# MCV-Univalle/HM-OpenCL

Hardware: AMD Instinct MI355X
Metric: GSAD/s (higher is better)
Workload: dtype u8

## Files before the change

### hm-opencl_amd/csrc/hmme.hip

```cpp
#include "../../include/hmme.h"
#include "../../include/hmme_test.h"

#include <hip/hip_runtime.h>

#include <climits>
#include <cmath>
#include <cstdarg>
#include <cstdio>
#include <cstdlib>
#include <cstring>
#include <functional>
#include <string>
#include <type_traits>
#include <vector>

#include "me_kernels.hpp"

using hmme::MeJob;
using hmme::MeJob16;
using hmme::RefSet;

namespace {
constexpr int kMarginX = 128;
constexpr int kMarginY = 80;
// ... 1225 lines not shown
    const int h = hmme::me_strip_rows16(w, w, rmax, n_min + 4);
    pl.n_strips = (w + h - 1) / h;
    const int lanes = (((w + 1) >> 1) + 2) / 3;
    auto strip_cost = [&](int k) {
      const int hk = (w + k - 1) / k;
      return 2.0 * ((((hk * lanes + 63) >> 6) + 3) >> 2) + 1.0;
    };
    if (tail && knobs.tail_parts != 1) {
      const int k_max = std::min(w / 4, 64);
      int k = knobs.tail_parts > 1 ? std::min(knobs.tail_parts, k_max) : plan_tail(tail, slots, pl.n_strips, k_max, strip_cost);
      if (k < pl.n_strips) k = pl.n_strips;
      if (k > pl.n_strips) { pl.tail_first = jobs - tail; pl.tail_parts = k; }
    }
    pl.n_wg16 = pl.tail_first * pl.n_strips + (jobs - pl.tail_first) * pl.tail_parts;
    pl.table_bytes = sizeof(MeJob16) * (size_t)pl.n_wg16;
  } else if (search_range > 64) {
    pl.mode = SearchMode::kTiles8;
    pl.table_bytes = sizeof(MeJob16) * (size_t)jobs * 4;
  } else {
    const int wgs = tail && knobs.tail_parts != 1 ? plan_tail8(tail, slots, w, knobs.tail_parts) : 0;
    if (wgs > 0) { pl.tail_first = jobs - tail; pl.tail_wgs = wgs; }
    const int head = pl.tail_first, n_tail = jobs - head;
    if (!n_tail) {
      pl.table_bytes = sizeof(MeJob) * (size_t)head;
    } else if (tail_one_launch(head, n_tail, knobs.tail_launches)) {
      pl.mode = SearchMode::kSegments8;
      pl.table_bytes = hmme::me_seg_table_bytes(head + wgs, jobs);
    } else {
      pl.mode = SearchMode::kHeadThenSegments8;
      pl.tail_jobs_off = (sizeof(MeJob) * (size_t)head + 255) & ~(size_t)255;
      pl.table_bytes = pl.tail_jobs_off + hmme::me_seg_table_bytes(wgs, n_tail);
    }
  }
  pl.first_strip = pl.mode != SearchMode::kWhole8;
  const size_t per_ref = n_refs > 0 ? (pl.table_bytes + n_refs - 1) / n_refs : pl.table_bytes;
  pl.table_grow = per_ref * hmme::kMaxRefs + 4096;
  return pl;
}
static FramePlan plan_launch(const hmme_ctx* ctx, const hmme_frame_params* fp, int count, int n_refs, bool force16 = false) {
  return plan_search(count * n_refs, n_refs, ctx->wg_slots, fp->search_range, fp->bit_depth > 8 || force16, knobs());
}

int hmme_test_tail_plan(int width, int height, int search_range, int n_pairs, int slots, int* out) {
  if (!out || width < 8 || height < 8 || width > 16384 || height > 16384 || search_range < 1 || search_range > 64 || n_pairs < 1 || slots < 1) return HMME_ERR_ARG;
  const FramePlan pl = plan_search(hmme_num_ctus(width, height) * n_pairs, n_pairs, slots, search_range, false, Knobs{});
  out[0] = pl.jobs; out[1] = pl.tail_first; out[2] = pl.tail_wgs; out[3] = pl.mode == SearchMode::kSegments8 ? 1 : 0;
  return HMME_OK;
}

int hmme_test_pk_gate(uint32_t lambda_q16) { return hmme::me_pk_gate(lambda_q16) ? 1 : 0; }
int hmme_test_pk_body(uint32_t lambda_q16, int fen) { return hmme::me_pk_body(lambda_q16, fen ? 1 : 0); }
int hmme_test_pk_task_marker_free(int wx, int wy, int k, int it0, int n_it) { return hmme::me_task_marker_free(wx, wy, k, it0, n_it) ? 1 : 0; }
int hmme_test_pk_task_full(int wx, int wy, int k, int it0, int n_it) { return hmme::me_task_full(wx, wy, k, it0, n_it) ? 1 : 0; }

static int prep_jobs(hmme_ctx* ctx, const hmme_plane* cur, const hmme_frame_params* fp, const void* d_pred_q, int first, int count,
                     int n_refs, hipStream_t s, const FramePlan& pl, const void* d_center_q = nullptr) {
  const int jobs = pl.jobs, head = pl.tail_first, n_tail = jobs - head, w = cur->width, h = cur->height, sr = fp->search_range;
  bool moved;
  int rc = ensure(ctx, ctx->buf[kJobs], pl.table_bytes, pl.table_grow, &moved);
  if (moved) ctx->jobs_tag.valid = false;
  if (rc) return rc;
  if (pl.first_strip) {
    rc = ensure(ctx, ctx->buf[kFirstStrip], sizeof(int) * (size_t)jobs, sizeof(int) * (size_t)(jobs / (n_refs > 0 ? n_refs : 1) + 1) * hmme::kMaxRefs, &moved);
    if (moved) ctx->jobs_tag.valid = false;
    if (rc) return rc;
  }
  void* const d_jobs = ctx->buf[kJobs].p;
  int* const d_first_strip = ctx->buf[kFirstStrip].as<int>();
  hmme_ctx::TableTag tag;
  tag.valid = !d_pred_q && !d_center_q;
  tag.w = w; tag.h = h; tag.sr = sr; tag.first = first; tag.count = count; tag.pairs = n_refs;
  tag.bit_depth = fp->bit_depth | (pl.mode == SearchMode::kStrips16 && fp->bit_depth == 8 ? 0x100 : 0);
  tag.buf = d_jobs; tag.buf2 = pl.first_strip ? d_first_strip : nullptr; tag.stream = (void*)s;
  if (tag.same(ctx->jobs_tag)) return HMME_OK;
  ctx->jobs_tag.valid = false;
  const dim3 block(256);
  const auto grid = [](int n) { return dim3((n + 255) / 256); };
  const int16_t* pred = (const int16_t*)d_pred_q;
  switch (pl.mode) {
    case SearchMode::kTiles8:
      hipLaunchKernelGGL(hmme::me_prep_jobs_tile_kernel, grid(jobs), block, 0, s, (MeJob16*)d_jobs, d_first_strip, pred, first, count, n_refs, w, h, sr);
      break;
    case SearchMode::kStrips16:
      hipLaunchKernelGGL(hmme::me_prep_jobs16_kernel, grid(jobs), block, 0, s, (MeJob16*)d_jobs, d_first_strip, pred, first, count, n_refs, w, h, sr,
                         pl.n_strips, pl.strip_rows, pl.tail_first, pl.tail_parts, (const int16_t*)d_center_q);
      break;
    case SearchMode::kWhole8:
    case SearchMode::kSegments8:
    case SearchMode::kHeadThenSegments8: {
      const int idx0 = pl.mode == SearchMode::kSegments8 ? head : 0;
      if (head && idx0)
        hipLaunchKernelGGL(hmme::me_prep_whole_segments_kernel, grid(head), block, 0, s, d_jobs, d_first_strip, pred, first, count, n_refs, w, h, sr,
                           head + pl.tail_wgs, head);
      else if (head)
        hipLaunchKernelGGL(hmme::me_prep_jobs_kernel, grid(head), block, 0, s, (MeJob*)d_jobs, pred, first, count, n_refs, w, h, sr, 0, head, 1,
                           (uint32_t*)nullptr, (const int16_t*)nullptr);
      if (n_tail)
        hipLaunchKernelGGL(hmme::me_prep_segments_kernel, dim3(1), dim3(hmme::kSegPrepThreads), 0, s, (void*)((uint8_t*)d_jobs + pl.tail_jobs_off), d_first_strip,
                           pred, first, count, n_refs, w, h, sr, idx0 + pl.tail_wgs, head, n_tail, idx0);
      break;
    }
  }
  HIP_TRY(ctx, hipGetLastError());
  ctx->jobs_tag = tag;
  return HMME_OK;
}
// ... 2671 lines not shown
```

### hm-opencl_amd/csrc/me_kernels.hpp

```cpp
#pragma once

#include <hip/hip_runtime.h>
#include <stdint.h>

namespace hmme {

constexpr int kParts = 593;
constexpr int kPDW = 49;
constexpr int kWinRowsMax = 192;
constexpr int kIdxBits = 10;
constexpr uint32_t kInvCost = 3146751u;
constexpr int kGroups = 10;
constexpr int kIterPerTask = 4;
constexpr int kIterPerTaskSplit = 1;
static_assert(kIterPerTask == 4 && kIterPerTaskSplit <= 4, "2 iteration bits in the key; the guided schedule deals 4 / 2 / 1");
constexpr int kThreads = 256;

struct MeJob {
  int16_t ctu_x, ctu_y;
  int16_t lt_x, lt_y;
  int16_t rb_x, rb_y;
  int16_t pred_x, pred_y;
};
static_assert(sizeof(MeJob) == 16, "MeJob layout");
// ... 35 lines not shown
  asm volatile("v_add3_u32 %0, %1, %2, %3" : "=v"(v##_3) : "v"(a##_3), "v"(b##_3), "v"(nc3))
#define ME_SUB(v, a, b)                                                                                         \
  uint32_t v##_0, v##_1, v##_2, v##_3;                                                                          \
  asm volatile("v_sad_u32 %0, %1, %2, %3" : "=v"(v##_0) : "v"(a##_0), "v"(b##_0), "v"(c0));                                \
  asm volatile("v_sad_u32 %0, %1, %2, %3" : "=v"(v##_1) : "v"(a##_1), "v"(b##_1), "v"(c1));                                \
  asm volatile("v_sad_u32 %0, %1, %2, %3" : "=v"(v##_2) : "v"(a##_2), "v"(b##_2), "v"(c2));                                \
  asm volatile("v_sad_u32 %0, %1, %2, %3" : "=v"(v##_3) : "v"(a##_3), "v"(b##_3), "v"(c3))
__device__ __forceinline__ uint32_t me_min4(uint32_t a, uint32_t b, uint32_t c, uint32_t d) {
  uint32_t r;
  asm volatile("v_min3_u32 %0, %1, %2, %3\n\tv_min_u32 %0, %0, %4" : "=&v"(r) : "v"(a), "v"(b), "v"(c), "v"(d));
  return r;
}
#define ME_MIN4(k) me_min4(k##_0, k##_1, k##_2, k##_3)
#define ME_SUBMIN4(r, a, b)                                                                                     \
  uint32_t r;                                                                                                   \
  {                                                                                                             \
    uint32_t r##_t, r##_u;                                                                                      \
    asm volatile("v_sad_u32 %0, %3, %7, %11\n\tv_sad_u32 %1, %4, %8, %12\n\tv_sad_u32 %2, %5, %9, %13\n\t"            \
                 "v_min3_u32 %0, %0, %1, %2\n\tv_sad_u32 %1, %6, %10, %14\n\tv_min_u32 %0, %0, %1"                    \
                 : "=&v"(r), "=&v"(r##_t), "=&v"(r##_u)                                                        \
                 : "v"(a##_0), "v"(a##_1), "v"(a##_2), "v"(a##_3), "v"(b##_0), "v"(b##_1), "v"(b##_2), "v"(b##_3), "v"(c0), "v"(c1),     \
                   "v"(c2), "v"(c3));                                                                           \
  }

constexpr uint32_t kPkSlotMax = 64 * 255;
constexpr uint32_t kPkMarker = 0xFFFFu - kPkSlotMax;
constexpr uint32_t kPkMaxBits = 2 * 37;
__host__ __device__ inline bool me_pk_gate(uint32_t lambda_q16) {
  const uint64_t prod = (uint64_t)lambda_q16 * kPkMaxBits;
  return prod <= 0xFFFFFFFFull && (prod >> 16) + kPkSlotMax < kPkMarker;
}
constexpr uint32_t kPk2SlotMax = 16 * 12 * 255;
__host__ __device__ inline bool me_pk2_gate(uint32_t lambda_q16) {
  const uint64_t prod = (uint64_t)lambda_q16 * kPkMaxBits;
  return prod <= 0xFFFFFFFFull && (prod >> 16) + kPk2SlotMax <= 0xFFFFu;
}
__host__ __device__ inline int me_pk_body(uint32_t lambda_q16, int fen) {
  return (fen && me_pk2_gate(lambda_q16)) ? 2 : me_pk_gate(lambda_q16) ? 1 : 0;
}
__host__ __device__ inline bool me_task_marker_free(int wx, int wy, int k, int it0, int n_it) {
  if (!(wx & 3)) return true;
  const int quads = (wx + 3) >> 2;
  if ((quads & -quads) == (1 << k)) return false;
  const bool fold = (quads & 32) && (quads & 31) && (wy & 1);
  return !(fold && k == 5 && 2 * (it0 + n_it) > wy);
}
__host__ __device__ inline bool me_task_full(int wx, int wy, int k, int it0, int n_it) {
  if (k < 2) return false;
  const int quads = (wx + 3) >> 2;
  if ((wx & 3) && (quads & -quads) == (1 << k)) return false;
  const bool fold = (quads & 32) && (quads & 31) && (wy & 1);
  return (it0 + n_it) * (64 >> k) <= ((k == 5 || !fold) ? wy : wy - 1);
}
#define ME_PKMIN(r, p) ME_PKMIN_Q(r, (p) + pkm)
#define ME_PKMINE(r, p) ME_PKMIN_Q(r, ((p) << 1) + pkm)
#define ME_PKMIN_Q(r, q)                                                                                        \
  uint32_t r;                                                                                                   \
  {                                                                                                             \
    const uint64_t r##_q = (q);                                                                                 \
    asm volatile("v_pk_min_u16 %0, %1, %2\n\tv_pk_min_u16 %0, %0, %0 op_sel:[0,1] op_sel_hi:[1,0]\n\t"                \
                 "v_mad_u32_u16 %0, %0, %3, %4"                                                                 \
                 : "=&v"(r) : "v"((uint32_t)r##_q), "v"((uint32_t)(r##_q >> 32)), "s"(mult_a), "v"(ctag));      \
  }

#define ME_PKMIN16_LO(r, q)                                                                                     \
  uint32_t r;                                                                                                   \
  {                                                                                                             \
    const uint64_t r##_q = (q);                                                                                 \
    asm volatile("v_pk_min_u16 %0, %1, %2\n\t"                                                                  \
                 "v_min_u16_sdwa %0, %0, %0 dst_sel:WORD_0 dst_unused:UNUSED_PAD src0_sel:WORD_0 src1_sel:WORD_1" \
                 : "=&v"(r) : "v"((uint32_t)r##_q), "v"((uint32_t)(r##_q >> 32)));                              \
  }
#define ME_PKMIN16_HI(r, q)                                                                                     \
  {                                                                                                             \
    const uint64_t r##_q = (q);                                                                                 \
    uint32_t r##_t;                                                                                             \
    asm volatile("v_pk_min_u16 %1, %2, %3\n\t"                                                                  \
                 "v_min_u16_sdwa %0, %1, %1 dst_sel:WORD_1 dst_unused:UNUSED_PRESERVE src0_sel:WORD_0 src1_sel:WORD_1" \
                 : "+v"(r), "=&v"(r##_t) : "v"((uint32_t)r##_q), "v"((uint32_t)(r##_q >> 32)));                 \
  }
#define ME_KEY16_LO(k, r) uint32_t k; asm volatile("v_mad_u32_u16 %0, %1, %2, %3" : "=v"(k) : "v"(r), "s"(mult_a), "v"(ctag))
#define ME_KEY16_HI(k, r) uint32_t k; asm volatile("v_mad_u32_u16 %0, %1, %2, %3 op_sel:[1,0,0,0]" : "=v"(k) : "v"(r), "s"(mult_a), "v"(ctag))
#define ME_PMERGE(NAME, PAD, SWAP)                                                                           \
  __device__ __forceinline__ uint32_t NAME(uint32_t a, uint32_t b) {                                         \
    asm volatile(PAD SWAP " %0, %1\n\tv_pk_min_u16 %0, %0, %1" : "+v"(a), "+v"(b));                          \
    return a;                                                                                                \
  }
ME_PMERGE(me_pmerge2, "s_nop 1\n\t", "v_permlane32_swap_b32")
ME_PMERGE(me_pmerge3, "s_nop 1\n\t", "v_permlane16_swap_b32")
ME_PMERGE(me_pmerge2_nn, "", "v_permlane32_swap_b32")
ME_PMERGE(me_pmerge3_nn, "", "v_permlane16_swap_b32")

#define ME_MERGE_DPP_MASKED(NAME, PAD, CTRL, MASK0)                                                          \
  __device__ __forceinline__ uint32_t NAME(uint32_t a, uint32_t b) {                                         \
    uint32_t r;                                                                                              \
    asm volatile(PAD "v_min_u32_dpp %0, %2, %2 " CTRL " row_mask:0xf bank_mask:0xf\n\t"                     \
        "v_min_u32_dpp %0, %1, %1 " CTRL " row_mask:0xf bank_mask:" MASK0                                    \
        : "=&v"(r) : "v"(a), "v"(b));                                                                        \
    return r;                                                                                                \
  }
ME_MERGE_DPP_MASKED(me_merge0, "s_nop 1\n\t", "row_ror:8", "0x3")
ME_MERGE_DPP_MASKED(me_merge1, "s_nop 1\n\t", "row_half_mirror", "0x5")
ME_MERGE_DPP_MASKED(me_merge0_nn, "", "row_ror:8", "0x3")
ME_MERGE_DPP_MASKED(me_merge1_nn, "", "row_half_mirror", "0x5")
__device__ __forceinline__ uint32_t me_merge2(uint32_t a, uint32_t b) {
  u32x2_t r = __builtin_amdgcn_permlane32_swap(a, b, false, false);
  return min(r.x, r.y);
}
__device__ __forceinline__ uint32_t me_merge3(uint32_t a, uint32_t b) {
  u32x2_t r = __builtin_amdgcn_permlane16_swap(a, b, false, false);
  return min(r.x, r.y);
}
template <int DPP_CTRL>
__device__ __forceinline__ uint32_t me_merge_dpp(uint32_t a, uint32_t b, bool role) {
  const uint32_t keep = role ? b : a;
  const uint32_t give = role ? a : b;
  return min(keep, (uint32_t)__builtin_amdgcn_update_dpp(0, (int)give, DPP_CTRL, 0xf, 0xf, false));
}
#define me_merge4(a, b, role) me_merge_dpp<0x4E>(a, b, role)
#define me_merge5(a, b, role) me_merge_dpp<0xB1>(a, b, role)

__device__ __forceinline__ uint32_t me_component_bits(int v) {
  const uint32_t t = (v <= 0) ? ((uint32_t)(-v) << 1) + 1u : ((uint32_t)v << 1);
  return 2u * (31u - (uint32_t)__builtin_clz(t)) + 1u;
}
__device__ __forceinline__ uint32_t me_mv_cost(uint32_t lambda_q16, int x, int y, int pred_x, int pred_y) {
  return (lambda_q16 * (me_component_bits((x << 2) - pred_x) + me_component_bits((y << 2) - pred_y))) >> 16;
}

__device__ __forceinline__ bool me_pk_slot(int s, bool wide, int& x, int& y, int& w, int& h) {
  if (s < 128) { x = (s & 7) * 8; y = (s >> 4) * 8 + ((s >> 3) & 1) * 4; w = 8; h = 4; return true; }
  if (s < 256) { x = ((s >> 1) & 7) * 8 + (s & 1) * 4; y = ((s - 128) >> 4) * 8; w = 4; h = 8; return true; }
  if (s >= 384 && s < 448) { x = (s & 7) * 8; y = ((s - 384) >> 3) * 8; w = 8; h = 8; return true; }
  if (!wide) return false;
  if (s < 384) {
    const int kk = (s - 256) >> 4;
    x = (s & 3) * 16; y = ((s >> 2) & 3) * 16; w = 16; h = 16;
    if (kk < 4) { h = kk < 2 ? 4 : 12; if (kk & 1) y += 16 - h; }
    else { w = kk < 6 ? 4 : 12; if (kk & 1) x += 16 - w; }
    return true;
  }
  if (s < 480) { x = (s & 3) * 16; y = ((s - 448) >> 3) * 16 + ((s >> 2) & 1) * 8; w = 16; h = 8; return true; }
  if (s < 512) { x = ((s >> 1) & 3) * 16 + (s & 1) * 8; y = ((s - 480) >> 3) * 16; w = 8; h = 16; return true; }
  return false;
}
template <int RW, int NR, int STEP>
__device__ __forceinline__ void me_pk_sads(const uint32_t* wrow, int pdw, const uint8_t* __restrict__ crow, uint32_t sad[4]) {
  constexpr int ND = RW / 4;
  static_assert(RW * NR * 255 <= 0xFFFF, "the four sums are packed u16");
  typedef uint64_t __attribute__((aligned(4))) u64a4_t;
  uint32_t c[NR][ND];
  uint64_t d[NR][ND];
#pragma unroll
  for (int r = 0; r < NR; ++r) {
#pragma unroll
    for (int k = 0; k < ND; ++k) c[r][k] = *(const uint32_t*)(crow + r * STEP * 64 + 4 * k);
#pragma unroll
    for (int k = 0; k < ND; ++k) d[r][k] = *(const u64a4_t*)(wrow + r * STEP * pdw + k);
  }
  uint64_t acc = 0;
#pragma unroll
  for (int r = 0; r < NR; ++r)
#pragma unroll
    for (int k = 0; k < ND; ++k) acc = ME_QSAD(d[r][k], c[r][k], acc);
#pragma unroll
  for (int j = 0; j < 4; ++j) sad[j] = (uint32_t)(acc >> (16 * j)) & 0xFFFFu;
}
template <bool WIDE>
__device__ __forceinline__ unsigned long long me_pk_recover(unsigned long long v, int s, const uint32_t* win, int pdw, const uint8_t* __restrict__ cur_blk,
                                                            const MeJob& job, int wx, uint32_t lambda_q16) {
  int rx, ry, rw, rh;
  if (v == ~0ull || !me_pk_slot(s, WIDE, rx, ry, rw, rh)) return v;
  const int x_first = (int)(v & 0xfffc), y = (int)((v >> 16) & 0xffff);
  const uint32_t cost = (uint32_t)(v >> 32);
  const uint8_t* crow = cur_blk + ry * 64 + rx;
  const uint32_t by = me_component_bits(((job.lt_y + y) << 2) - job.pred_y);
  const int x_end = (WIDE && !(x_first & 12)) ? min(x_first + 16, wx) : x_first + 4;
// ... 169 lines not shown
    if (!first_job) __syncthreads();
  }
  if (fair_prio) __builtin_amdgcn_s_setprio(3);
  const uint8_t* __restrict__ ref_base = refs.base[job.ctu_x & 63];
  const uint8_t* __restrict__ cur_base = curs.base[job.ctu_x & 63];
  job.ctu_x &= ~63;
  const int wx = job.rb_x - job.lt_x + 1, wy = job.rb_y - job.lt_y + 1;

  for (int s = tid; s < kParts; s += kThreads) best64[s] = ~0ull;
  if (tid == 0) task_ctr = t_first;

  const uintptr_t cur_addr = (uintptr_t)(cur_base + ((long)(job.ctu_y >> 6) * cur_ctus_x + (job.ctu_x >> 6)) * kBlkBytes8);
  const uint64_t curc = (uint64_t)(uint32_t)__builtin_amdgcn_readfirstlane((uint32_t)cur_addr) |
                        (uint64_t)(uint32_t)__builtin_amdgcn_readfirstlane((uint32_t)(cur_addr >> 32)) << 32;
  if (tid < 64) me_prefetch_cur<1>(curc);
  {
    const uint8_t* src = ref_base + (long)(job.ctu_y + job.lt_y) * ref_pitch + (job.ctu_x + job.lt_x);
    const uint32_t mis = (uint32_t)(uintptr_t)src & 3u;
    const uint32_t* src_al = (const uint32_t*)(src - mis);
    const int pitch_dw = ref_pitch >> 2;
    const int n = (wy + 63) * kPDW;
    me_stage_window<kPDW, kThreads>(win, src_al, pitch_dw, n, mis, tid);
  }
  __syncthreads();
#ifdef ME_SEARCH_T_TIMELINE
  const unsigned long long tl_staged = wall_clock64();
#endif

  const int quads = (wx + 3) >> 2;
  constexpr int kIt = SPLIT ? kIterPerTaskSplit : kIterPerTask;
  constexpr bool kGuided = !SPLIT;
  const int n_tasks = kGuided ? me_num_tasks_guided(wx, wy) : min(me_num_tasks(wx, wy, kIt), t_end);
  const bool fold = me_fold(quads, wy);
  const int wy_low = fold ? wy - 1 : wy;

  const uint32_t mult_a = 1u << kIdxBits;
  const uint32_t mult_e = FEN ? (2u << kIdxBits) : (1u << kIdxBits);
  const bool rb1 = lane & 2, rb0 = lane & 1;
  int prio_quarter = 0x0fffffff;
  if (fair_prio) {
    if constexpr (!SPLIT) {
      int total = 0;
      for (int kk = 5; kk >= 0; --kk)
        if (quads & (1 << kk)) total += ((kk == 5 ? wy : wy_low) + (64 >> kk) - 1) / (64 >> kk);
      prio_quarter = max(1, (total + 15) >> 4);
    } else {
      prio_quarter = max(1, ((n_tasks - t_first) * kIt + 15) >> 4);
    }
  }
  int prio_state = prio_quarter << 2;

  static_assert(SPLIT != 2 || kIterPerTaskSplit == 1, "segment mode counts tasks in lane-iterations");
  int grab_next = 0, grab_end = 0;
  while (true) {
    int t = 0;
    if constexpr (SPLIT == 2) {
      if (grab_next >= grab_end) {
        int want = 0;
        if (lane == 0) {
          const int left = n_tasks - *(volatile int*)&task_ctr;
          want = min(4, max(1, (left + 3) >> 2));
          t = atomicAdd(&task_ctr, want);
        }
        t = __builtin_amdgcn_readfirstlane(t);
        want = __builtin_amdgcn_readfirstlane(want);
        if (t >= n_tasks) break;
        grab_next = t; grab_end = min(t + want, n_tasks);
      }
      t = grab_next;
    } else {
      if (lane == 0) t = atomicAdd(&task_ctr, 1);
      t = __builtin_amdgcn_readfirstlane(t);
      if (t >= n_tasks) break;
    }
    if (prio_state < 4 && (prio_state & 3) < 3) {
      prio_state += (prio_quarter << 2) + 1;
      if ((prio_state & 3) == 1) __builtin_amdgcn_s_setprio(2);
      else if ((prio_state & 3) == 2) __builtin_amdgcn_s_setprio(1);
      else __builtin_amdgcn_s_setprio(0);
    }
    int x0 = 0, k = 0, it0 = 0, n_it = 0;
    {
      int xq = 0, rem = t;
      for (int kk = 5; kk >= 0; --kk) {
        if (!(quads & (1 << kk))) continue;
        const int iters = ((kk == 5 ? wy : wy_low) + (64 >> kk) - 1) / (64 >> kk);
        int nt;
        if constexpr (kGuided) {
          int n4, n2, n1;
          me_guided(iters, n4, n2, n1);
          nt = n4 + n2 + n1;
          if (rem < nt) {
            x0 = xq * 4; k = kk;
            if (rem < n4) { it0 = 4 * rem; n_it = 4; }
            else if (rem < n4 + n2) { it0 = 4 * n4 + 2 * (rem - n4); n_it = 2; }
            else { it0 = 4 * n4 + 2 * n2 + (rem - n4 - n2); n_it = 1; }
            break;
          }
        } else {
          nt = (iters + kIt - 1) / kIt;
          if (rem < nt) {
            x0 = xq * 4; k = kk; it0 = rem * kIt; n_it = min(kIt, iters - it0);
            if constexpr (SPLIT == 2) { n_it = min(grab_end - grab_next, iters - it0); grab_next += n_it; }
            break;
          }
        }
        rem -= nt;
        xq += 1 << kk;
      }
    }
    const int ty = 64 >> k;
    const bool full = PK == 2 && me_task_full(wx, wy, k, it0, n_it);
    int lx = lane & ((1 << k) - 1), ly = lane >> k;
    if (full) { lx = ((lane >> 5) & 1) | ((lane >> 3) & 2) | ((lane & ((1 << (k - 2)) - 1)) << 2); ly = (lane & 15) >> (k - 2); }
    const bool fold_part = fold && k == 5;

    uint32_t b0 = ME_MAXKEY, b1 = ME_MAXKEY, b2 = ME_MAXKEY, b3 = ME_MAXKEY, b4 = ME_MAXKEY, b5 = ME_MAXKEY,
             b6 = ME_MAXKEY, b7 = ME_MAXKEY, b8 = ME_MAXKEY, b9 = ME_MAXKEY;

    prio_state -= n_it << 2;
    for (int it = 0; it < n_it; ++it) {
      int cx = x0 + 4 * lx, cy = (it0 + it) * ty + ly;
      if (fold_part && cy == wy) { cx += 128; cy = wy - 1; }
      const bool vy = cy < wy;
      const int mvy = job.lt_y + cy, mvx = job.lt_x + cx;
      const uint32_t by = me_component_bits((mvy << 2) - job.pred_y);
      uint32_t lane_now = (uint32_t)(ly << k | lx);
      asm("" : "+v"(lane_now));
      const uint32_t tag = ((uint32_t)it << 8) | (lane_now << 2);
      uint32_t cc[4];
#pragma unroll
      for (int j = 0; j < 4; ++j) {
        const uint32_t cost = (lambda_q16 * (me_component_bits(((mvx + j) << 2) - job.pred_x) + by)) >> 16;
        cc[j] = (((vy && (cx + j) < wx) ? cost : kInvCost) << kIdxBits) | tag | (uint32_t)j;
      }
      const uint32_t c0 = cc[0], c1 = cc[1], c2 = cc[2], c3 = cc[3];
      const uint32_t nc0 = 0u - c0, nc1 = 0u - c1, nc2 = 0u - c2, nc3 = 0u - c3;
      uint64_t pkm = 0;
      uint32_t ctag = 0;
      if constexpr (PK) {
        const uint32_t m0 = cc[0] < (kInvCost << kIdxBits) ? cc[0] >> kIdxBits : kPkMarker, m1 = cc[1] < (kInvCost << kIdxBits) ? cc[1] >> kIdxBits : kPkMarker;
        const uint32_t m2 = cc[2] < (kInvCost << kIdxBits) ? cc[2] >> kIdxBits : kPkMarker, m3 = cc[3] < (kInvCost << kIdxBits) ? cc[3] >> kIdxBits : kPkMarker;
        pkm = (uint64_t)(m0 | m1 << 16) | (uint64_t)(m2 | m3 << 16) << 32;
        ctag = ((vy && cx < wx) ? 0u : kInvCost << kIdxBits) | tag;
        if (full) ctag = tag & ~(3u << 2);
      }
      uint64_t npkm = 0;
      if constexpr (PK == 2) {
        npkm = 0ull - pkm;
        asm volatile("" : "+v"(npkm));
      }
      const lds_char_t* lpc = (const lds_char_t*)(win + min(cy, wy - 1) * kPDW + (min(cx, wx - 1) >> 2));
#define ME8_CUR(row, q)                                                                                                            \
  ({                                                                                                                               \
    uint64_t w_;                                                                                                                   \
    asm volatile("s_load_dwordx2 %0, %1, %2" : "=s"(w_) : "s"(curc), "n"((row) * 64 + 8 * (q)));                                    \
    w_;                                                                                                                            \
  })
#define ME8_CUR_WAIT(w0, w1, w2, w3, w4, w5, w6, w7, d0, d1, d2, d3, d4, d5, d6, d7, d8, d9, d10, d11, d12, d13, d14, d15)           \
  asm volatile("" : : "v"(d0), "v"(d1), "v"(d2), "v"(d3), "v"(d4), "v"(d5), "v"(d6), "v"(d7), "v"(d8), "v"(d9), "v"(d10), "v"(d11),  \
               "v"(d12), "v"(d13), "v"(d14), "v"(d15));                                                                             \
  asm volatile("s_waitcnt lgkmcnt(0)" : "+s"(w0), "+s"(w1), "+s"(w2), "+s"(w3), "+s"(w4), "+s"(w5), "+s"(w6), "+s"(w7))
      if constexpr (PK == 2) {
        static_assert(PK != 2 || FEN == 1, "the full-task body exists for FEN 1");
        if (full) {
#include "me_tree_pk4_fen1.inc"
        } else {
#include "me_tree_pk_fen1.inc"
        }
      } else if constexpr (PK) {
        if constexpr (FEN) {
#include "me_tree_pk_fen1.inc"
        } else {
#include "me_tree_pk_fen0.inc"
        }
      } else if constexpr (FEN) {
#include "me_tree_fen1.inc"
      } else {
#include "me_tree_fen0.inc"
      }
    }

#define ME_FLUSH(g, key_)                                                                                          \
    {                                                                                                              \
      const int slot = full ? ME_SLOT_OF3[g][lane] : ME_SLOT_OF[g][lane];                                          \
      const uint32_t key = (key_);                                                                                 \
      const uint32_t cost = key >> kIdxBits;                                                                       \
      if (slot >= 0 && cost < kInvCost) {                                                                          \
        const int kit = (key >> 8) & 3, kl = (key >> 2) & 63, kj = key & 3;                                        \
        int bx = x0 + 4 * (kl & ((1 << k) - 1)) + kj;                                                              \
        int byy = (it0 + kit) * ty + (kl >> k);                                                                    \
        if (fold_part && byy == wy) { bx += 128; byy = wy - 1; }                                                   \
        atomicMin(&best64[slot],                                                                                   \
                  ((unsigned long long)cost << 32) | ((unsigned long long)byy << 16) | (unsigned long long)bx);    \
      }                                                                                                            \
    }
    ME_FLUSH(0, b0) ME_FLUSH(1, b1) ME_FLUSH(2, b2) ME_FLUSH(3, b3) ME_FLUSH(4, b4)
    ME_FLUSH(5, b5) ME_FLUSH(6, b6) ME_FLUSH(7, b7) ME_FLUSH(8, b8) ME_FLUSH(9, b9)
#undef ME_FLUSH
  }
#ifdef ME_SEARCH_T_TIMELINE
  const unsigned long long tl_dry = wall_clock64();
#endif
  __syncthreads();
#ifdef ME_SEARCH_T_TIMELINE
  const unsigned long long tl_all = wall_clock64();
#endif

  if constexpr (SPLIT) {
    for (int s = tid; s < kParts; s += kThreads) {
      unsigned long long v = best64[s];
      if constexpr (PK) v = me_pk_recover<PK == 2>(v, s, win, kPDW, (const uint8_t*)cur_addr, job, wx, lambda_q16);
      if (v != ~0ull) atomicMin(&g_best[(long)out_job * kParts + s], v + tile_off);
    }
    if constexpr (SPLIT == 2) {
      if (seg_g < seg_end) continue;
    }
    return;
  }
  for (int s = tid; s < kParts; s += kThreads) {
    unsigned long long v = best64[s];
    if constexpr (PK) v = me_pk_recover<PK == 2>(v, s, win, kPDW, (const uint8_t*)cur_addr, job, wx, lambda_q16);
    const int mvx = job.lt_x + (int)(v & 0xffff), mvy = job.lt_y + (int)((v >> 16) & 0xffff);
    const uint32_t cost = (uint32_t)(v >> 32);
    const long o = (long)out_job * kParts + s;
    out_mv[2 * o] = (int16_t)mvx;
    out_mv[2 * o + 1] = (int16_t)mvy;
    out_sad[o] = cost - me_mv_cost(lambda_q16, mvx, mvy, job.pred_x, job.pred_y);
  }
#ifdef ME_SEARCH_T_TIMELINE
  __syncthreads();
  if (lane == 0) {
    uint32_t* o = out_sad + (long)out_job * kParts;
    const int wv = tid >> 6;
    if (wv == 0) {
      const unsigned long long t1 = wall_clock64();
      uint32_t hw_id;
      asm volatile("s_getreg_b32 %0, hwreg(HW_REG_HW_ID)" : "=s"(hw_id));
      uint32_t xcc_id;
      asm volatile("s_getreg_b32 %0, hwreg(HW_REG_XCC_ID)" : "=s"(xcc_id));
      o[0] = (uint32_t)tl_start; o[1] = (uint32_t)(tl_start >> 32); o[2] = (uint32_t)(tl_staged - tl_start); o[3] = (uint32_t)(tl_all - tl_start);
      o[4] = (uint32_t)(t1 - tl_start); o[5] = hw_id; o[6] = xcc_id; o[7] = blockIdx.x;
    }
    o[8 + wv] = (uint32_t)(tl_dry - tl_start);
  }
#endif
  break;
  }
}


// ... 2570 lines not shown
```

### hm-opencl_amd/hmme/api.py

```python
import ctypes as C
import os
import subprocess

import numpy as np

HERE = os.path.dirname(os.path.abspath(__file__))
CSRC = os.path.join(os.path.dirname(HERE), "csrc")
LIB_PATH = os.environ.get("HMME_LIB", os.path.join(CSRC, "libhmme.so"))
NUM_PARTS = 593

SYMBOLS = ["hmme_create", "hmme_destroy", "hmme_last_error", "hmme_device_info", "hmme_set_lambda",
           "hmme_set_lambda_q16", "hmme_get_lambda_q16", "hmme_params_ocl_compat", "hmme_set_search_range",
           "hmme_slot_index", "hmme_slot_rect", "hmme_slot_index_amp_off", "hmme_amp_off_slot", "hmme_compact_amp_off", "hmme_search_ctu", "hmme_search_ctu_w", "hmme_search_refine_ctu_w", "hmme_refine_ctu_w", "hmme_search_refine_ctu", "hmme_refine_ctu", "hmme_plane_create", "hmme_plane_create_ex", "hmme_plane_bit_depth", "hmme_plane_destroy", "hmme_plane_upload_pel",
           "hmme_plane_upload_u8", "hmme_host_register", "hmme_host_unregister", "hmme_plane_set_device_u8", "hmme_plane_width", "hmme_plane_height",
           "hmme_num_ctus", "hmme_search_frame", "hmme_search_frame_device", "hmme_search_frame_multi",
           "hmme_search_frame_multi_device", "hmme_refine_frame", "hmme_refine_frame_multi_device",
           "hmme_search_pairs_device", "hmme_refine_pairs_device", "hmme_plane_upload_async",
           "hmme_upload_status", "hmme_abi_version", "hmme_build_id", "hmme_device_index", "hmme_set_error_printing",
           "hmme_weight_check", "hmme_search_pairs_w_device", "hmme_refine_pairs_w_device", "hmme_search_frame_w", "hmme_refine_frame_w",
           "hmme_bipred_check", "hmme_predict_pairs_device", "hmme_predict_frame", "hmme_search_pairs_bi_device", "hmme_refine_pairs_bi_device",
           "hmme_search_frame_bi", "hmme_refine_frame_bi",
           "hmme_bipred_weight_check", "hmme_predict_pairs_w_device", "hmme_predict_frame_w", "hmme_search_pairs_bi_w_device",
           "hmme_refine_pairs_bi_w_device", "hmme_search_frame_bi_w", "hmme_refine_frame_bi_w",
           "hmme_slot_key", "hmme_select_check", "hmme_select_pairs_device", "hmme_select_frame",
           "hmme_ref_idx_bits", "hmme_select_refs_check", "hmme_select_refs_device", "hmme_select_refs_frame",
           "hmme_predict_refs_device", "hmme_predict_refs_frame",
           "hmme_select_dirs_check", "hmme_select_dirs_device", "hmme_select_dirs_frame", "hmme_predict_bi_device", "hmme_predict_bi_frame",
           "hmme_predict_bi_weight_check", "hmme_predict_bi_w_device", "hmme_predict_bi_w_frame", "hmme_predict_refs_w_device", "hmme_predict_refs_w_frame",
           "hmme_plane_stats", "hmme_wp_estimate", "hmme_wp_estimate_420",
           "hmme_predict_chroma_pairs_device", "hmme_predict_chroma_frame", "hmme_predict_chroma_refs_device", "hmme_predict_chroma_refs_frame",
           "hmme_predict_refs4_device", "hmme_predict_refs4_frame", "hmme_predict_chroma_refs4_device", "hmme_predict_chroma_refs4_frame",
           "hmme_predict_chroma_bi_device", "hmme_predict_chroma_bi_frame",
           "hmme_residual_pairs_device", "hmme_residual_frame",
           "hmme_search_frame_bi_refs_device", "hmme_refine_frame_bi_refs_device", "hmme_search_frame_bi_refs", "hmme_refine_frame_bi_refs",
           "hmme_select_dirs_refs_check", "hmme_select_dirs_refs_device", "hmme_select_dirs_refs_frame",
           "hmme_predict_bi_refs_device", "hmme_predict_bi_refs_frame",
           "hmme_bipred_refs_weight_check", "hmme_search_frame_bi_refs_w_device", "hmme_refine_frame_bi_refs_w_device", "hmme_search_frame_bi_refs_w",
           "hmme_refine_frame_bi_refs_w",
           "hmme_predict_bi_refs_weight_check", "hmme_predict_bi_refs_w_device", "hmme_predict_bi_refs_w_frame",
           "hmme_predict_chroma_bi_refs_device", "hmme_predict_chroma_bi_refs_frame",
           "hmme_search_pairs_bi4_device", "hmme_refine_pairs_bi4_device", "hmme_search_frame_bi4", "hmme_refine_frame_bi4",
           "hmme_select_dirs4_check", "hmme_select_dirs4_device", "hmme_select_dirs4_frame",
           "hmme_predict_bi4_device", "hmme_predict_bi4_frame", "hmme_predict_chroma_bi4_device", "hmme_predict_chroma_bi4_frame",
           "hmme_search_frame_bi_refs4_device", "hmme_refine_frame_bi_refs4_device", "hmme_search_frame_bi_refs4", "hmme_refine_frame_bi_refs4",
           "hmme_select_dirs_refs4_check", "hmme_select_dirs_refs4_device", "hmme_select_dirs_refs4_frame",
           "hmme_predict_bi_refs4_device", "hmme_predict_bi_refs4_frame", "hmme_predict_chroma_bi_refs4_device", "hmme_predict_chroma_bi_refs4_frame"]
TEST_SYMBOLS = ["hmme_test_time_search_kernel", "hmme_test_device_address", "hmme_test_frac_deal", "hmme_test_tail_plan", "hmme_test_stage_layout", "hmme_test_picture_job", "hmme_test_time_weight_passes", "hmme_test_time_bipred_origin",
                "hmme_test_time_wp_estimate_passes", "hmme_test_pk_gate", "hmme_test_pk_body", "hmme_test_pk_task_marker_free", "hmme_test_pk_task_full",
                "hmme_test_wp_parameters", "hmme_test_wp_select", "hmme_test_ctu_plan"]
ABI_VERSION = 6


class HmmeError(RuntimeError):
    pass


class SearchParams(C.Structure):
    _fields_ = [("lt_x", C.c_int), ("lt_y", C.c_int), ("rb_x", C.c_int), ("rb_y", C.c_int),
                ("pred_x", C.c_int), ("pred_y", C.c_int), ("fen", C.c_int), ("bit_depth", C.c_int),
                ("shift_free", C.c_int)]


class Weight(C.Structure):
    _fields_ = [("w0", C.c_int), ("offset", C.c_int), ("shift", C.c_int), ("round", C.c_int)]


class WpInfo(C.Structure):
    _fields_ = [("cur_dc_sum", C.c_int64), ("cur_ac", C.c_int64), ("ref_dc_sum", C.c_int64), ("ref_ac", C.c_int64),
                ("sad_wp", C.c_int64), ("sad_nowp", C.c_int64),
                ("log2_denom", C.c_int), ("weight", C.c_int), ("offset", C.c_int), ("present", C.c_int),
                ("served_search", C.c_int), ("served_refine", C.c_int)]

    def as_dict(self):
        return {k: int(getattr(self, k)) for k, _ in self._fields_}


class SelectParams(C.Structure):
    _fields_ = [("mv_per_ctu", C.c_int), ("mv_unit", C.c_int), ("price_mv", C.c_int), ("part_mask", C.c_uint),
                ("min_depth", C.c_int), ("max_depth", C.c_int), ("cu_cost", C.c_uint32), ("pu_cost", C.c_uint32)]

    def __init__(self, mv_per_ctu=64, mv_unit=0, price_mv=0, part_mask=0xF7, min_depth=0, max_depth=3, cu_cost=0, pu_cost=0):
        super().__init__(int(mv_per_ctu), int(mv_unit), int(price_mv), int(part_mask), int(min_depth), int(max_depth), int(cu_cost), int(pu_cost))


class DirParams(C.Structure):
    _fields_ = [("dir_bits", C.c_uint32 * 3), ("list_bits", C.c_uint32 * 2)]

    def __init__(self, dir_bits=(0, 0, 0), list_bits=(0, 0)):
        super().__init__((C.c_uint32 * 3)(*[int(v) for v in dir_bits]), (C.c_uint32 * 2)(*[int(v) for v in list_bits]))


class DirRefsParams(C.Structure):
    _fields_ = [("dir_bits", C.c_uint32 * 3), ("n_refs", C.c_int * 2), ("ref_bits", (C.c_uint32 * 8) * 2), ("l1_valid_mask", C.c_uint32)]

    def __init__(self, dir_bits=(0, 0, 0), n_refs=(1, 1), ref_bits=((), ()), l1_valid_mask=None):
        rb = ((C.c_uint32 * 8) * 2)()
        for l in range(2):
            for r, v in enumerate(ref_bits[l]):
                rb[l][r] = int(v)
        mask = (1 << int(n_refs[1])) - 1 if l1_valid_mask is None else int(l1_valid_mask)
        super().__init__((C.c_uint32 * 3)(*[int(v) for v in dir_bits]), (C.c_int * 2)(*[int(v) for v in n_refs]), rb, mask)
# ... 1295 lines not shown
```

Baseline: 4127.

## Carry per-lane best keys across consecutive full tasks and precompute full-task costs

In the packed-min full-task search path, the running best keys b0..b7 are kept across consecutive tasks that share the same partition size and column, instead of being flushed to global memory with atomicMin after every task. The carried key encodes the absolute row and group so it can be decoded at flush time. Each lane's per-column MV bit costs are also computed once per task, and the per-iteration cost and negation use packed perm and v_xad instructions. This removes repeated global atomics and per-iteration cost arithmetic, in exchange for more live registers, an extra loop iteration for draining, and a limit on row index range that the new carry_fits helper checks.

```diff
diff --git a/hm-opencl_amd/csrc/hmme.hip b/hm-opencl_amd/csrc/hmme.hip
--- a/hm-opencl_amd/csrc/hmme.hip
+++ b/hm-opencl_amd/csrc/hmme.hip
@@ -1301,6 +1301,16 @@
 int hmme_test_pk_body(uint32_t lambda_q16, int fen) { return hmme::me_pk_body(lambda_q16, fen ? 1 : 0); }
 int hmme_test_pk_task_marker_free(int wx, int wy, int k, int it0, int n_it) { return hmme::me_task_marker_free(wx, wy, k, it0, n_it) ? 1 : 0; }
 int hmme_test_pk_task_full(int wx, int wy, int k, int it0, int n_it) { return hmme::me_task_full(wx, wy, k, it0, n_it) ? 1 : 0; }
+int hmme_test_task_carry_fits(int wx, int wy, int k, int it0, int n_it) { return hmme::me_task_carry_fits(wx, wy, k, it0, n_it) ? 1 : 0; }
+int hmme_test_carry_index(int k, int row, int group) {
+  if (k < 2 || k > 5 || row < 0 || group < 0 || group >= 1 << (k - 2)) return -1;
+  return (int)hmme::me_carry_index(k, row, group);
+}
+int hmme_test_carry_position(int k, int index, int* out) {
+  if (k < 2 || k > 5 || index < 0 || index >= 1 << hmme::kIdxBits || !out) return -1;
+  hmme::me_carry_position(k, (uint32_t)index, out[0], out[1]);
+  return 0;
+}
 
 static int prep_jobs(hmme_ctx* ctx, const hmme_plane* cur, const hmme_frame_params* fp, const void* d_pred_q, int first, int count,
                      int n_refs, hipStream_t s, const FramePlan& pl, const void* d_center_q = nullptr) {
diff --git a/hm-opencl_amd/csrc/me_kernels.hpp b/hm-opencl_amd/csrc/me_kernels.hpp
--- a/hm-opencl_amd/csrc/me_kernels.hpp
+++ b/hm-opencl_amd/csrc/me_kernels.hpp
@@ -111,6 +111,19 @@
   const bool fold = (quads & 32) && (quads & 31) && (wy & 1);
   return (it0 + n_it) * (64 >> k) <= ((k == 5 || !fold) ? wy : wy - 1);
 }
+constexpr int kCarryGroupBits = 4, kCarryItBits = kIdxBits - kCarryGroupBits;
+__host__ __device__ inline bool me_task_carry_fits(int wx, int wy, int k, int it0, int n_it) {
+  return !me_task_full(wx, wy, k, it0, n_it) || it0 + n_it <= (1 << kCarryItBits);
+}
+__host__ __device__ inline uint32_t me_carry_index(int k, int row, int group) {
+  const int ty = 64 >> k;
+  return (uint32_t)((row / ty) << kCarryGroupBits | (row % ty) << (k - 2) | group);
+}
+__host__ __device__ inline void me_carry_position(int k, uint32_t index, int& row, int& group) {
+  const int g4 = (int)(index & ((1u << kCarryGroupBits) - 1));
+  row = (int)(index >> kCarryGroupBits) * (64 >> k) + (g4 >> (k - 2));
+  group = g4 & ((1 << (k - 2)) - 1);
+}
 #define ME_PKMIN(r, p) ME_PKMIN_Q(r, (p) + pkm)
 #define ME_PKMINE(r, p) ME_PKMIN_Q(r, ((p) << 1) + pkm)
 #define ME_PKMIN_Q(r, q)                                                                                        \
@@ -182,6 +195,17 @@
 __device__ __forceinline__ uint32_t me_component_bits(int v) {
   const uint32_t t = (v <= 0) ? ((uint32_t)(-v) << 1) + 1u : ((uint32_t)v << 1);
   return 2u * (31u - (uint32_t)__builtin_clz(t)) + 1u;
+}
+__device__ __forceinline__ uint32_t me_neg_xad(uint32_t x) {
+  uint32_t r;
+  asm("v_xad_u32 %0, %1, -1, 1" : "=v"(r) : "v"(x));
+  return r;
+}
+__device__ __forceinline__ uint32_t me_component_bits_xad(int v) {
+  const uint32_t v2 = (uint32_t)v << 1;
+  uint32_t t;
+  asm("v_xad_u32 %0, %1, -1, 2" : "=v"(t) : "v"(v2));
+  return 2u * (31u - (uint32_t)__builtin_clz(v > 0 ? v2 : t)) + 1u;
 }
 __device__ __forceinline__ uint32_t me_mv_cost(uint32_t lambda_q16, int x, int y, int pred_x, int pred_y) {
   return (lambda_q16 * (me_component_bits((x << 2) - pred_x) + me_component_bits((y << 2) - pred_y))) >> 16;
@@ -457,6 +481,10 @@
 
   static_assert(SPLIT != 2 || kIterPerTaskSplit == 1, "segment mode counts tasks in lane-iterations");
   int grab_next = 0, grab_end = 0;
+  constexpr bool kCarry = PK == 2 && SPLIT == 0;
+  uint32_t b0 = ME_MAXKEY, b1 = ME_MAXKEY, b2 = ME_MAXKEY, b3 = ME_MAXKEY, b4 = ME_MAXKEY, b5 = ME_MAXKEY,
+           b6 = ME_MAXKEY, b7 = ME_MAXKEY, b8 = ME_MAXKEY, b9 = ME_MAXKEY;
+  int carry_k = -1, carry_x0 = 0;
   while (true) {
     int t = 0;
     if constexpr (SPLIT == 2) {
@@ -476,8 +504,9 @@
     } else {
       if (lane == 0) t = atomicAdd(&task_ctr, 1);
       t = __builtin_amdgcn_readfirstlane(t);
-      if (t >= n_tasks) break;
-    }
+      if (!kCarry && t >= n_tasks) break;
+    }
+    const bool dry = t >= n_tasks;
     if (prio_state < 4 && (prio_state & 3) < 3) {
       prio_state += (prio_quarter << 2) + 1;
       if ((prio_state & 3) == 1) __builtin_amdgcn_s_setprio(2);
@@ -516,46 +545,44 @@
     }
     const int ty = 64 >> k;
     const bool full = PK == 2 && me_task_full(wx, wy, k, it0, n_it);
-    int lx = lane & ((1 << k) - 1), ly = lane >> k;
-    if (full) { lx = ((lane >> 5) & 1) | ((lane >> 3) & 2) | ((lane & ((1 << (k - 2)) - 1)) << 2); ly = (lane & 15) >> (k - 2); }
     const bool fold_part = fold && k == 5;
 
-    uint32_t b0 = ME_MAXKEY, b1 = ME_MAXKEY, b2 = ME_MAXKEY, b3 = ME_MAXKEY, b4 = ME_MAXKEY, b5 = ME_MAXKEY,
-             b6 = ME_MAXKEY, b7 = ME_MAXKEY, b8 = ME_MAXKEY, b9 = ME_MAXKEY;
-
-    prio_state -= n_it << 2;
-    for (int it = 0; it < n_it; ++it) {
-      int cx = x0 + 4 * lx, cy = (it0 + it) * ty + ly;
-      if (fold_part && cy == wy) { cx += 128; cy = wy - 1; }
-      const bool vy = cy < wy;
-      const int mvy = job.lt_y + cy, mvx = job.lt_x + cx;
-      const uint32_t by = me_component_bits((mvy << 2) - job.pred_y);
-      uint32_t lane_now = (uint32_t)(ly << k | lx);
-      asm("" : "+v"(lane_now));
-      const uint32_t tag = ((uint32_t)it << 8) | (lane_now << 2);
-      uint32_t cc[4];
-#pragma unroll
-      for (int j = 0; j < 4; ++j) {
-        const uint32_t cost = (lambda_q16 * (me_component_bits(((mvx + j) << 2) - job.pred_x) + by)) >> 16;
-        cc[j] = (((vy && (cx + j) < wx) ? cost : kInvCost) << kIdxBits) | tag | (uint32_t)j;
-      }
-      const uint32_t c0 = cc[0], c1 = cc[1], c2 = cc[2], c3 = cc[3];
-      const uint32_t nc0 = 0u - c0, nc1 = 0u - c1, nc2 = 0u - c2, nc3 = 0u - c3;
-      uint64_t pkm = 0;
-      uint32_t ctag = 0;
-      if constexpr (PK) {
-        const uint32_t m0 = cc[0] < (kInvCost << kIdxBits) ? cc[0] >> kIdxBits : kPkMarker, m1 = cc[1] < (kInvCost << kIdxBits) ? cc[1] >> kIdxBits : kPkMarker;
-        const uint32_t m2 = cc[2] < (kInvCost << kIdxBits) ? cc[2] >> kIdxBits : kPkMarker, m3 = cc[3] < (kInvCost << kIdxBits) ? cc[3] >> kIdxBits : kPkMarker;
-        pkm = (uint64_t)(m0 | m1 << 16) | (uint64_t)(m2 | m3 << 16) << 32;
-        ctag = ((vy && cx < wx) ? 0u : kInvCost << kIdxBits) | tag;
-        if (full) ctag = tag & ~(3u << 2);
-      }
-      uint64_t npkm = 0;
-      if constexpr (PK == 2) {
-        npkm = 0ull - pkm;
-        asm volatile("" : "+v"(npkm));
-      }
-      const lds_char_t* lpc = (const lds_char_t*)(win + min(cy, wy - 1) * kPDW + (min(cx, wx - 1) >> 2));
+    if constexpr (kCarry) {
+      if (carry_k >= 0 && !(full && k == carry_k && x0 == carry_x0)) {
+#define ME_FLUSH_CARRIED(g, key_)                                                                                  \
+        {                                                                                                          \
+          const int slot = ME_SLOT_OF3[g][lane];                                                                   \
+          const uint32_t key = (key_);                                                                             \
+          const uint32_t cost = key >> kIdxBits;                                                                   \
+          if (slot >= 0 && cost < kInvCost) {                                                                      \
+            int row, group;                                                                                        \
+            me_carry_position(carry_k, key & ((1u << kIdxBits) - 1), row, group);                                  \
+            atomicMin(&best64[slot], ((unsigned long long)cost << 32) | ((unsigned long long)row << 16) |          \
+                                         (unsigned long long)(carry_x0 + 16 * group));                             \
+          }                                                                                                        \
+        }
+        ME_FLUSH_CARRIED(0, b0) ME_FLUSH_CARRIED(1, b1) ME_FLUSH_CARRIED(2, b2) ME_FLUSH_CARRIED(3, b3)
+        ME_FLUSH_CARRIED(4, b4) ME_FLUSH_CARRIED(5, b5) ME_FLUSH_CARRIED(6, b6) ME_FLUSH_CARRIED(7, b7)
+#undef ME_FLUSH_CARRIED
+        carry_k = -1;
+      }
+      if (dry) break;
+    }
+    if (carry_k < 0) b0 = b1 = b2 = b3 = b4 = b5 = b6 = b7 = ME_MAXKEY;
+    b8 = b9 = ME_MAXKEY;
+
+    uint32_t f_bx = 0, f_tag = 0;
+    int f_vy = 0;
+    const lds_char_t* f_lpc = (const lds_char_t*)win;
+    if (full) {
+      const int lx = ((lane >> 5) & 1) | ((lane >> 3) & 2) | ((lane & ((1 << (k - 2)) - 1)) << 2), ly = (lane & 15) >> (k - 2);
+      const int cx = x0 + 4 * lx, cy = it0 * ty + ly;
+      const int vx = ((job.lt_x + cx) << 2) - job.pred_x;
+      f_bx = me_component_bits(vx) | me_component_bits(vx + 4) << 8 | me_component_bits(vx + 8) << 16 | me_component_bits(vx + 12) << 24;
+      f_tag = (uint32_t)(ly << k | lx) << 2;
+      f_vy = ((job.lt_y + cy) << 2) - job.pred_y;
+      f_lpc = (const lds_char_t*)(win + cy * kPDW + (cx >> 2));
+    }
 #define ME8_CUR(row, q)                                                                                                            \
   ({                                                                                                                               \
     uint64_t w_;                                                                                                                   \
@@ -566,13 +593,58 @@
   asm volatile("" : : "v"(d0), "v"(d1), "v"(d2), "v"(d3), "v"(d4), "v"(d5), "v"(d6), "v"(d7), "v"(d8), "v"(d9), "v"(d10), "v"(d11),  \
                "v"(d12), "v"(d13), "v"(d14), "v"(d15));                                                                             \
   asm volatile("s_waitcnt lgkmcnt(0)" : "+s"(w0), "+s"(w1), "+s"(w2), "+s"(w3), "+s"(w4), "+s"(w5), "+s"(w6), "+s"(w7))
+
+    prio_state -= n_it << 2;
+    for (int it = 0; it < n_it; ++it) {
+      if (full) {
+        if constexpr (PK == 2) {
+          static_assert(PK != 2 || FEN == 1, "the full-task body exists for FEN 1");
+          const uint32_t by = me_component_bits_xad(f_vy + it * (4 * ty));
+          const uint32_t p0 = lambda_q16 * ((f_bx & 255u) + by), p1 = lambda_q16 * (((f_bx >> 8) & 255u) + by);
+          const uint32_t p2 = lambda_q16 * (((f_bx >> 16) & 255u) + by), p3 = lambda_q16 * ((f_bx >> 24) + by);
+          const uint64_t pkm = (uint64_t)__builtin_amdgcn_perm(p1, p0, 0x07060302u) | (uint64_t)__builtin_amdgcn_perm(p3, p2, 0x07060302u) << 32;
+          uint64_t npkm = ~pkm;
+          asm volatile("" : "+v"(npkm));
+          npkm += 1;
+          asm volatile("" : "+v"(npkm));
+          const uint32_t tag = ((uint32_t)it << 8) | f_tag;
+          const uint32_t ctag = kCarry ? (uint32_t)(it0 + it) << kCarryGroupBits | f_tag >> 4 : tag & ~(3u << 2);
+          const uint32_t c0 = (p0 >> 16) << kIdxBits | tag, c1 = (p1 >> 16) << kIdxBits | tag | 1u;
+          const uint32_t c2 = (p2 >> 16) << kIdxBits | tag | 2u, c3 = (p3 >> 16) << kIdxBits | tag | 3u;
+          const uint32_t nc0 = me_neg_xad(c0), nc1 = me_neg_xad(c1), nc2 = me_neg_xad(c2), nc3 = me_neg_xad(c3);
+          const lds_char_t* lpc = f_lpc + it * (ty * kPDW * 4);
+#include "me_tree_pk4_fen1.inc"
+        }
+        continue;
+      }
+      uint32_t lane_now = (uint32_t)lane;
+      asm("" : "+v"(lane_now));
+      const int lx = lane_now & ((1 << k) - 1), ly = lane_now >> k;
+      int cx = x0 + 4 * lx, cy = (it0 + it) * ty + ly;
+      if (fold_part && cy == wy) { cx += 128; cy = wy - 1; }
+      const bool vy = cy < wy;
+      const int mvy = job.lt_y + cy, mvx = job.lt_x + cx;
+      const uint32_t by = me_component_bits((mvy << 2) - job.pred_y);
+      const uint32_t tag = ((uint32_t)it << 8) | (lane_now << 2);
+      uint32_t cc[4];
+#pragma unroll
+      for (int j = 0; j < 4; ++j) {
+        const uint32_t cost = (lambda_q16 * (me_component_bits(((mvx + j) << 2) - job.pred_x) + by)) >> 16;
+        cc[j] = (((vy && (cx + j) < wx) ? cost : kInvCost) << kIdxBits) | tag | (uint32_t)j;
+      }
+      const uint32_t c0 = cc[0], c1 = cc[1], c2 = cc[2], c3 = cc[3];
+      const uint32_t nc0 = 0u - c0, nc1 = 0u - c1, nc2 = 0u - c2, nc3 = 0u - c3;
+      uint64_t pkm = 0;
+      uint32_t ctag = 0;
+      if constexpr (PK) {
+        const uint32_t m0 = cc[0] < (kInvCost << kIdxBits) ? cc[0] >> kIdxBits : kPkMarker, m1 = cc[1] < (kInvCost << kIdxBits) ? cc[1] >> kIdxBits : kPkMarker;
+        const uint32_t m2 = cc[2] < (kInvCost << kIdxBits) ? cc[2] >> kIdxBits : kPkMarker, m3 = cc[3] < (kInvCost << kIdxBits) ? cc[3] >> kIdxBits : kPkMarker;
+        pkm = (uint64_t)(m0 | m1 << 16) | (uint64_t)(m2 | m3 << 16) << 32;
+        ctag = ((vy && cx < wx) ? 0u : kInvCost << kIdxBits) | tag;
+      }
+      const lds_char_t* lpc = (const lds_char_t*)(win + min(cy, wy - 1) * kPDW + (min(cx, wx - 1) >> 2));
       if constexpr (PK == 2) {
-        static_assert(PK != 2 || FEN == 1, "the full-task body exists for FEN 1");
-        if (full) {
-#include "me_tree_pk4_fen1.inc"
-        } else {
 #include "me_tree_pk_fen1.inc"
-        }
       } else if constexpr (PK) {
         if constexpr (FEN) {
 #include "me_tree_pk_fen1.inc"
@@ -600,8 +672,13 @@
                   ((unsigned long long)cost << 32) | ((unsigned long long)byy << 16) | (unsigned long long)bx);    \
       }                                                                                                            \
     }
-    ME_FLUSH(0, b0) ME_FLUSH(1, b1) ME_FLUSH(2, b2) ME_FLUSH(3, b3) ME_FLUSH(4, b4)
-    ME_FLUSH(5, b5) ME_FLUSH(6, b6) ME_FLUSH(7, b7) ME_FLUSH(8, b8) ME_FLUSH(9, b9)
+    if (!(kCarry && full)) {
+      ME_FLUSH(0, b0) ME_FLUSH(1, b1) ME_FLUSH(2, b2) ME_FLUSH(3, b3)
+      ME_FLUSH(4, b4) ME_FLUSH(5, b5) ME_FLUSH(6, b6) ME_FLUSH(7, b7)
+    } else {
+      carry_k = k; carry_x0 = x0;
+    }
+    ME_FLUSH(8, b8) ME_FLUSH(9, b9)
 #undef ME_FLUSH
   }
 #ifdef ME_SEARCH_T_TIMELINE
diff --git a/hm-opencl_amd/hmme/api.py b/hm-opencl_amd/hmme/api.py
--- a/hm-opencl_amd/hmme/api.py
+++ b/hm-opencl_amd/hmme/api.py
@@ -47,6 +47,7 @@
            "hmme_predict_bi_refs4_device", "hmme_predict_bi_refs4_frame", "hmme_predict_chroma_bi_refs4_device", "hmme_predict_chroma_bi_refs4_frame"]
 TEST_SYMBOLS = ["hmme_test_time_search_kernel", "hmme_test_device_address", "hmme_test_frac_deal", "hmme_test_tail_plan", "hmme_test_stage_layout", "hmme_test_picture_job", "hmme_test_time_weight_passes", "hmme_test_time_bipred_origin",
                 "hmme_test_time_wp_estimate_passes", "hmme_test_pk_gate", "hmme_test_pk_body", "hmme_test_pk_task_marker_free", "hmme_test_pk_task_full",
+                "hmme_test_task_carry_fits", "hmme_test_carry_index", "hmme_test_carry_position",
                 "hmme_test_wp_parameters", "hmme_test_wp_select", "hmme_test_ctu_plan"]
 ABI_VERSION = 6
 
```

New measurement: 4173, median of 6. 1.01x the previous value.
